# tachitachi/SR-WaveNet

Hardware: AMD Instinct MI355X
Metric: audio samples/sec (fwd+bwd) 30-layer teacher WaveNet (higher is better)
Workload: dtype bf16; 1 GPU; 30-layer teacher WaveNet (3x[1..512] dilations, 64 res / 256 skip ch, 256-way mu-law softmax), fwd+bwd+Adam, batch 8x16000 samples per GPU; global_batch=8, seq_len=16000, parallelism=dp1, launch=hipGraph

## Files before the change

### sr-wavenet_amd/csrc/srwn_wgradt.hip

```cpp
#include "srwn_common.h"
#include "srwn_group.h"
#include "srwn_host.h"
#include "../../include/srwn.h"

using namespace srwn;
using namespace srwn::grp;

namespace {

constexpr int kMaxBlk = 16;
constexpr int kNB = 4;
constexpr int kTileB = 32 * 512;

struct WtBlk { int nl; int layer[4]; int st, W, nsub, KT; };
struct WtSkipArgs {
  const void* cT; long long wt_stride;
  const void* d; long long d_row_stride;
  void* partials; float* bias_partials;
  int part16;
  int B, Tlen, nslabs, mtotal;
  int safe_wait;
  int bias_blk;
  WtBlk blk[kMaxBlk];
};

__device__ uint4 g_zero_row[32];

typedef bf16_t T;

__device__ __forceinline__ f32x4 gload16_untracked(const void* p) {
  f32x4 v;
  asm volatile("global_load_dwordx4 %0, %1, off nt" : "=v"(v) : "v"(p) : "memory");
  return v;
}

struct Cursor {
  int idx, seg, k, wrem;
  long long drow0;
};

__global__ __launch_bounds__(512) void wgrad_skip_wt_kernel(WtSkipArgs a) {
  extern __shared__ __attribute__((aligned(16))) char smem[];
  const int tid = threadIdx.x, lane = tid & 63, wave = __builtin_amdgcn_readfirstlane(tid >> 6);
  const int slab = blockIdx.x;
  const WtBlk& bk = a.blk[blockIdx.y];
  const int st = bk.st, W = bk.W, nsub = bk.nsub, KT = bk.KT;
  const int slot = wave >> 1, nh = wave & 1;
  const bool live = slot < bk.nl;
  const int layer = bk.layer[live ? slot : 0];
  const int per_clip = st * nsub;
  const int nseg = a.B * per_clip;
  const int sps = (nseg + a.nslabs - 1) / a.nslabs;
  const int s0 = slab * sps;
  const int s1 = (s0 + sps < nseg) ? s0 + sps : nseg;
  const int nchunk = (s1 > s0 ? s1 - s0 : 0) * KT;
  const int nit = (nchunk + 2) / 3 * 3;

  auto seg_setup = [&](Cursor& c) {
    const int b = c.seg / per_clip;
    const int rem = c.seg - b * per_clip;
    int r, j0;
    if (nsub == 1) { r = rem; j0 = 0; }
    else { r = rem / nsub; j0 = (rem - r * nsub) * W; }
    const int Jr = (a.Tlen - r + st - 1) / st;
    const int wseg = (Jr - j0) < W ? (Jr - j0) : W;
    c.wrem = wseg;
    c.drow0 = (long long)b * a.Tlen + r + (long long)st * j0;
  };
  auto start = [&](Cursor& c) {
    c.idx = 0; c.seg = nchunk > 0 ? s0 : 0; c.k = 0; c.wrem = 0; c.drow0 = 0;
    if (nchunk > 0) seg_setup(c);
  };
  auto advance = [&](Cursor& c) {
    ++c.idx;
    if (c.idx >= nchunk) { c.wrem = 0; return; }
    ++c.k; c.wrem -= 32;
    if (c.k == KT) { c.k = 0; ++c.seg; seg_setup(c); }
  };

  const int drow_a = 2 * wave + (lane >> 5);
  const int dcol = 32 * ((((lane & 31) >> 1) ^ wave)) + 16 * (lane & 1);
  const char* dbase = reinterpret_cast<const char*>(a.d) + dcol;
  const char* zrow = reinterpret_cast<const char*>(g_zero_row) + dcol;
  const long long drow_bytes = a.d_row_stride * (long long)sizeof(T);
  const unsigned lds0 = (unsigned)(size_t)smem;
  auto dma_tile = [&](const Cursor& c, int buf) {
    const long long row0 = c.drow0 + (long long)st * (32 * c.k);
    const char* ga = (drow_a < c.wrem) ? dbase + (row0 + (long long)st * drow_a) * drow_bytes : zrow;
    const char* gb = (drow_a + 16 < c.wrem) ? dbase + (row0 + (long long)st * (drow_a + 16)) * drow_bytes : zrow;
    const unsigned l = lds0 + buf * kTileB + wave * 1024;
    glds16_untracked(ga, __builtin_amdgcn_readfirstlane(l));
    glds16_untracked(gb, __builtin_amdgcn_readfirstlane(l + 8 * 1024));
  };
  const T* ct_layer = reinterpret_cast<const T*>(a.cT) + (size_t)layer * a.wt_stride + lane * 8;
  auto load_a = [&](const Cursor& c, f32x4 (&f)[4]) {
    const T* t = ct_layer + ((size_t)c.seg * KT + c.k) * (64 * 32);
#pragma unroll
    for (int mb = 0; mb < 4; ++mb) f[mb] = gload16_untracked(t + mb * 512);
  };

  const int kg = lane >> 4, q = (lane & 15) >> 2, p = lane & 3;
  const int hl = ((kg & 1) + 2 * q) & 7;
  const int rowoff = (16 * (kg >> 1) + 2 * (kg & 1) + 4 * q) * 512 + 8 * p;
  int boff[8];
#pragma unroll
  for (int i = 0; i < 8; ++i) boff[i] = rowoff + 32 * (8 * nh + (i ^ hl));

  f32x4 acc[4][8];
#pragma unroll
  for (int mb = 0; mb < 4; ++mb)
#pragma unroll
    for (int i = 0; i < 8; ++i) acc[mb][i] = f32x4{0.f, 0.f, 0.f, 0.f};
  const bool do_bias = a.bias_partials != nullptr && (int)blockIdx.y == a.bias_blk && slot == 3;
  float bsum[8];
#pragma unroll
  for (int i = 0; i < 8; ++i) bsum[i] = 0.0f;
  Frag<T> ones;
#pragma unroll
  for (int j = 0; j < 8; ++j) ones.set(j, 1.0f);

  Cursor ca, cd;
  start(ca); start(cd);
  f32x4 A0[4], A1[4], A2[4];
  dma_tile(cd, 0); advance(cd);
  load_a(ca, A0); advance(ca);
  dma_tile(cd, 1); advance(cd);
  load_a(ca, A1); advance(ca);
  dma_tile(cd, 2); advance(cd);

  typedef short s16x4 __attribute__((ext_vector_type(4)));
  auto bfrag = [&](int buf, int i) {
    const char* bp = smem + buf * kTileB + boff[i];
    s16x4 lo = __builtin_amdgcn_ds_read_tr16_b64_v4i16((__attribute__((address_space(3))) s16x4*)(bp));
    s16x4 hi = __builtin_amdgcn_ds_read_tr16_b64_v4i16((__attribute__((address_space(3))) s16x4*)(bp + 512));
    Frag<T> bf;
    bf.v = __builtin_bit_cast(bf16x8, __builtin_shufflevector(lo, hi, 0, 1, 2, 3, 4, 5, 6, 7));
    return bf;
  };
  Frag<T> bq0 = zero_frag<T>(), bq1 = zero_frag<T>();
  auto compute = [&](int buf, int nbuf, const f32x4 (&A)[4]) {
    Frag<T> af[4];
#pragma unroll
    for (int mb = 0; mb < 4; ++mb) af[mb].v = __builtin_bit_cast(bf16x8, A[mb]);
    Frag<T> b[10];
    b[0] = bq0; b[1] = bq1;
#pragma unroll
    for (int i = 0; i < 8; ++i) {
      b[i + 2] = (i + 2 < 8) ? bfrag(buf, i + 2) : bfrag(nbuf, i + 2 - 8);
#pragma unroll
      for (int mb = 0; mb < 4; ++mb) mma16(acc[mb][i], af[mb], b[i]);
      __builtin_amdgcn_sched_barrier(0);
    }
    bq0 = b[8]; bq1 = b[9];
  };
  auto bias_only = [&](int buf) {
#pragma unroll
    for (int i = 0; i < 8; ++i) bsum[i] = frag_dot(bsum[i], bfrag(buf, i), ones);
  };
#define SRWN_WT_ITER(IT, ACUR, ANEW)                                                                            \
  {                                                                                                             \
        \
    asm volatile("s_waitcnt vmcnt(6)" : "+v"(ACUR[0]), "+v"(ACUR[1]), "+v"(ACUR[2]), "+v"(ACUR[3])::"memory");       \
    if (a.safe_wait) asm volatile("s_waitcnt vmcnt(0)" : "+v"(ACUR[0]), "+v"(ACUR[1]), "+v"(ACUR[2]), "+v"(ACUR[3])::"memory"); \
    wg_barrier();                                                                                               \
    load_a(ca, ANEW); advance(ca);                                                                              \
    dma_tile(cd, ((IT) + 3) & (kNB - 1)); advance(cd);                                                          \
    if (live) compute((IT) & (kNB - 1), ((IT) + 1) & (kNB - 1), ACUR);                                          \
    else if (do_bias) bias_only((IT) & (kNB - 1));                                                              \
  }
  if (nit > 0) {
    if (a.safe_wait) asm volatile("s_waitcnt vmcnt(0)" ::: "memory");
    else asm volatile("s_waitcnt vmcnt(6)" ::: "memory");
    wg_barrier();
    if (live) { bq0 = bfrag(0, 0); bq1 = bfrag(0, 1); }
  }
  for (int it = 0; it < nit; it += 3) {
    SRWN_WT_ITER(it, A0, A2)
    SRWN_WT_ITER(it + 1, A1, A0)
    SRWN_WT_ITER(it + 2, A2, A1)
  }
#undef SRWN_WT_ITER
  asm volatile("s_waitcnt vmcnt(0)" : "+v"(A0[0]), "+v"(A1[0]), "+v"(A2[0])::"memory");

  if (live && a.part16) {
    bf16_t* pb = reinterpret_cast<bf16_t*>(a.partials) + (size_t)slab * a.mtotal * 256;
#pragma unroll
    for (int mb = 0; mb < 4; ++mb)
#pragma unroll
      for (int i = 0; i < 8; ++i) {
        const size_t blk = (size_t)(layer * 4 + mb) * 16 + 8 * nh + i;
        __builtin_nontemporal_store(bf16x4{(bf16_t)acc[mb][i][0], (bf16_t)acc[mb][i][1], (bf16_t)acc[mb][i][2], (bf16_t)acc[mb][i][3]},
                                    reinterpret_cast<bf16x4*>(pb + (blk * 64 + lane) * 4));
      }
  } else if (live) {
    float* pb = reinterpret_cast<float*>(a.partials) + ((size_t)slab * a.mtotal + (size_t)layer * 64) * 256 + 128 * nh + (lane & 15);
#pragma unroll
    for (int mb = 0; mb < 4; ++mb)
#pragma unroll
      for (int i = 0; i < 8; ++i)
#pragma unroll
        for (int r = 0; r < 4; ++r) pb[(size_t)(16 * mb + 4 * (lane >> 4) + r) * 256 + 16 * i] = acc[mb][i][r];
  }
  if (do_bias) {
#pragma unroll
    for (int i = 0; i < 8; ++i) {
      float v = bsum[i];
      v += __shfl_xor(v, 16);
      v += __shfl_xor(v, 32);
      if (lane < 16) a.bias_partials[(size_t)slab * 256 + 128 * nh + 16 * i + lane] = v;
    }
  }
}

__global__ __launch_bounds__(256) void colsum256_kernel(const T* d, long long row_stride, long long rows, int nslabs, float* out) {
  const long long rps = (rows + nslabs - 1) / nslabs;
  const long long r0 = (long long)blockIdx.x * rps;
  const long long r1 = (r0 + rps < rows) ? r0 + rps : rows;
  float s0 = 0.0f, s1 = 0.0f;
  const int c = 2 * (threadIdx.x & 127), half = threadIdx.x >> 7;
  for (long long r = r0 + half; r < r1; r += 2) {
    const unsigned v = *reinterpret_cast<const unsigned*>(d + r * row_stride + c);
    s0 += __builtin_bit_cast(float, v << 16);
    s1 += __builtin_bit_cast(float, v & 0xffff0000u);
  }
  __shared__ float red[2][256];
  red[half][c] = s0; red[half][c + 1] = s1;
  __syncthreads();
  out[(size_t)blockIdx.x * 256 + threadIdx.x] = red[0][threadIdx.x] + red[1][threadIdx.x];
}

int plan_blocks(const int32_t* st, const int32_t* seg_rows, int nlayers, int T, WtBlk* out) {
  int nb = 0;
  bool used[512] = {false};
  if (nlayers > 512) return -1;
  for (int l = 0; l < nlayers; ++l) {
    if (used[l]) continue;
    if (nb == kMaxBlk) return -1;
    WtBlk& b = out[nb++];
    b.nl = 0; b.st = st[l]; b.W = seg_rows[l];
    const int J = (T + b.st - 1) / b.st;
    b.nsub = (J + b.W - 1) / b.W;
    b.KT = (b.W + 31) / 32;
    for (int m = l; m < nlayers && b.nl < 4; ++m)
      if (!used[m] && st[m] == b.st && seg_rows[m] == b.W) { b.layer[b.nl++] = m; used[m] = true; }
    for (int i = b.nl; i < 4; ++i) b.layer[i] = b.layer[0];
  }
  return nb;
}

}

extern "C" int32_t srwn_wgrad_skip_wt_slabs(const int32_t* st, const int32_t* seg_rows, int32_t nlayers, int32_t T) {
  if (!st || !seg_rows || nlayers < 1 || T < 1) return 0;
  for (int l = 0; l < nlayers; ++l) if (st[l] < 1 || seg_rows[l] < 1) return 0;
  WtBlk blk[kMaxBlk];
  const int nb = plan_blocks(st, seg_rows, nlayers, T, blk);
  if (nb < 1) return 0;
  const int s = group_grid() / nb;
  return s < 1 ? 1 : s;
}

extern "C" int srwn_wgrad_skip_wt(const void* cT, int64_t wt_layer_stride, const int32_t* st, const int32_t* seg_rows,
                                  int32_t nlayers, const void* d, int64_t d_row_stride, void* partials,
                                  float* bias_partials, int32_t part16, int32_t nslabs, int32_t B, int32_t T, int32_t R,
                                  int32_t S, int32_t dtype, void* stream) {
  if (B == 0 || T == 0 || nlayers == 0) return 0;
  if (!cT || !st || !seg_rows || !d || !partials) return set_error(SRWN_E_NULL, "wgrad_skip_wt: null pointer");
  if (dtype != SRWN_BF16 || R != 64 || S != 256)
    return set_error(SRWN_E_UNSUPPORTED, "wgrad_skip_wt: built for bf16, 64 residual / 256 skip channels (dtype %d R=%d S=%d)", dtype, R, S);
  if (B < 0 || T < 0 || nlayers < 0 || nslabs < 1 || d_row_stride < S || (d_row_stride % 8) || wt_layer_stride < 0)
    return set_error(SRWN_E_SHAPE, "wgrad_skip_wt: B=%d T=%d layers=%d nslabs=%d d_row_stride=%lld", B, T, nlayers, nslabs,
                     (long long)d_row_stride);
  for (int l = 0; l < nlayers; ++l)
    if (st[l] < 1 || seg_rows[l] < 1) return set_error(SRWN_E_SHAPE, "wgrad_skip_wt: layer %d stride %d segment %d", l, st[l], seg_rows[l]);
  WtSkipArgs a;
  a.cT = cT; a.wt_stride = wt_layer_stride; a.d = d; a.d_row_stride = d_row_stride; a.partials = partials;
  a.part16 = part16 ? 1 : 0;
  a.bias_partials = bias_partials; a.B = B; a.Tlen = T; a.nslabs = nslabs; a.mtotal = nlayers * 64;
  const int nb = plan_blocks(st, seg_rows, nlayers, T, a.blk);
  if (nb < 1) return set_error(SRWN_E_UNSUPPORTED, "wgrad_skip_wt: more than %d layer blocks", kMaxBlk);
  for (int i = 0; i < nb; ++i) {
    const long long nseg = (long long)B * a.blk[i].st * a.blk[i].nsub;
    if (nseg > 0x7fffffffLL || nseg * a.blk[i].KT * 64 * 32 > wt_layer_stride)
      return set_error(SRWN_E_SHAPE, "wgrad_skip_wt: %lld segments x %d tiles exceed wt_layer_stride %lld", nseg, a.blk[i].KT,
                       (long long)wt_layer_stride);
  }
  a.bias_blk = -1;
  a.safe_wait = safe_wait();
  if (bias_partials)
    for (int i = 0; i < nb && a.bias_blk < 0; ++i)
      if (a.blk[i].nl < 4) a.bias_blk = i;
  if (bias_partials && a.bias_blk < 0)
    hipLaunchKernelGGL(colsum256_kernel, dim3((unsigned)nslabs), dim3(256), 0, (hipStream_t)stream,
                       reinterpret_cast<const bf16_t*>(d), (long long)d_row_stride, (long long)B * T, nslabs, bias_partials);
  const size_t sh = (size_t)kNB * kTileB;
  hipError_t e = hipFuncSetAttribute((const void*)wgrad_skip_wt_kernel, hipFuncAttributeMaxDynamicSharedMemorySize, (int)sh);
  if (e != hipSuccess) return set_error((int)e, "wgrad_skip_wt: LDS %zu: %s", sh, hipGetErrorString(e));
  hipLaunchKernelGGL(wgrad_skip_wt_kernel, dim3((unsigned)nslabs, (unsigned)nb), dim3(512), sh, (hipStream_t)stream, a);
  return check_launch("wgrad_skip_wt");
}
```

Before: 80.02 million samples/s.

## Stage A operand through LDS ring with spread DMA issue in wgrad skip kernel

Adds a default LDS mode where the cT (A) operand is DMA'd into a 5-slot LDS ring through global_load_lds instead of being held in three register sets. The next A fragment is read mid-compute, and the tile and A DMA issues are spread between MFMA steps. The aim is to cut register pressure and even out memory issue against the MFMA work. It costs more LDS (about 144KB in total), which may lower occupancy, and adds LDS read traffic. Alternative register modes and debug timestamp instrumentation are also added.

```diff
diff --git a/sr-wavenet_amd/csrc/srwn_wgradt.hip b/sr-wavenet_amd/csrc/srwn_wgradt.hip
--- a/sr-wavenet_amd/csrc/srwn_wgradt.hip
+++ b/sr-wavenet_amd/csrc/srwn_wgradt.hip
@@ -11,6 +11,22 @@
 constexpr int kMaxBlk = 16;
 constexpr int kNB = 4;
 constexpr int kTileB = 32 * 512;
+constexpr int kRing = 5;
+constexpr int kSlotB = 16 * 1024;
+constexpr int kStampB = 2 * 512 * 8;
+enum { kWtRegs3 = 0, kWtRegs4 = 1, kWtLds = 2 };
+#ifndef SRWN_WT_MODE
+#define SRWN_WT_MODE 2
+#endif
+constexpr int kWtMode = SRWN_WT_MODE;
+#ifndef SRWN_WT_SPREAD
+#define SRWN_WT_SPREAD 2
+#endif
+constexpr bool kWtSpread = SRWN_WT_SPREAD != 0;
+constexpr int kWtSpreadAt = SRWN_WT_SPREAD == 2 ? 4 : 0;
+constexpr size_t wt_lds_bytes(int mode, bool stamp) {
+  return (size_t)kNB * kTileB + (mode == kWtLds ? (size_t)kRing * kSlotB : 0) + (stamp ? kStampB : 0);
+}
 
 struct WtBlk { int nl; int layer[4]; int st, W, nsub, KT; };
 struct WtSkipArgs {
@@ -21,6 +37,7 @@
   int B, Tlen, nslabs, mtotal;
   int safe_wait;
   int bias_blk;
+  unsigned long long* stamps;
   WtBlk blk[kMaxBlk];
 };
 
@@ -34,14 +51,36 @@
   return v;
 }
 
+__device__ __forceinline__ void glds16_nt_untracked(const void* g, unsigned lds_addr) {
+  unsigned keep;
+  asm volatile("s_mov_b32 %0, m0\n\ts_mov_b32 m0, %2\n\ts_nop 0\n\tglobal_load_lds_dwordx4 %1, off nt\n\ts_mov_b32 m0, %0"
+               : "=&s"(keep) : "v"(g), "s"(lds_addr) : "memory");
+}
+
+template <bool STAMP> struct WtStamper {
+  unsigned long long* p; int n;
+  __device__ __forceinline__ void operator()(int tag) {
+    if (STAMP && p && n < 512) { p[n] = ((unsigned long long)tag << 48) | (__builtin_amdgcn_s_memtime() & 0xffffffffffffull); ++n; }
+  }
+};
+
 struct Cursor {
   int idx, seg, k, wrem;
   long long drow0;
 };
 
+template <int MODE, bool STAMP>
 __global__ __launch_bounds__(512) void wgrad_skip_wt_kernel(WtSkipArgs a) {
   extern __shared__ __attribute__((aligned(16))) char smem[];
   const int tid = threadIdx.x, lane = tid & 63, wave = __builtin_amdgcn_readfirstlane(tid >> 6);
+  WtStamper<STAMP> stamp{nullptr, 0};
+  const bool stamped = STAMP && blockIdx.x == 0 && blockIdx.y == 0 && (wave & 3) == 0;
+  unsigned long long* const stamp_lds = reinterpret_cast<unsigned long long*>(smem + wt_lds_bytes(MODE, false)) + (wave >> 2) * 512;
+  if (stamped) {
+    for (int i = lane; i < 512; i += 64) stamp_lds[i] = 0;
+    if (lane == 0) stamp.p = stamp_lds;
+  }
+  stamp(1);
   const int slab = blockIdx.x;
   const WtBlk& bk = a.blk[blockIdx.y];
   const int st = bk.st, W = bk.W, nsub = bk.nsub, KT = bk.KT;
@@ -54,7 +93,8 @@
   const int s0 = slab * sps;
   const int s1 = (s0 + sps < nseg) ? s0 + sps : nseg;
   const int nchunk = (s1 > s0 ? s1 - s0 : 0) * KT;
-  const int nit = (nchunk + 2) / 3 * 3;
+  constexpr int kSets = MODE == kWtRegs4 ? 4 : 3;
+  const int nit = MODE == kWtLds ? nchunk : (nchunk + kSets - 1) / kSets * kSets;
 
   auto seg_setup = [&](Cursor& c) {
     const int b = c.seg / per_clip;
@@ -84,17 +124,26 @@
   const char* zrow = reinterpret_cast<const char*>(g_zero_row) + dcol;
   const long long drow_bytes = a.d_row_stride * (long long)sizeof(T);
   const unsigned lds0 = (unsigned)(size_t)smem;
+  const char* dlane_a = dbase + (long long)st * drow_a * drow_bytes;
+  const char* dlane_b = dbase + (long long)st * (drow_a + 16) * drow_bytes;
+  struct TileDma { const char* ga; const char* gb; unsigned l; };
+  auto tile_addr = [&](const Cursor& c, int buf) {
+    const long long tile0 = (c.drow0 + (long long)st * (32 * c.k)) * drow_bytes;
+    TileDma t;
+    t.ga = (drow_a < c.wrem) ? dlane_a + tile0 : zrow;
+    t.gb = (drow_a + 16 < c.wrem) ? dlane_b + tile0 : zrow;
+    t.l = __builtin_amdgcn_readfirstlane(lds0 + buf * kTileB + wave * 1024);
+    return t;
+  };
+  auto dma_half = [&](const TileDma& t, int h) { glds16_untracked(h ? t.gb : t.ga, t.l + h * 8 * 1024); };
   auto dma_tile = [&](const Cursor& c, int buf) {
-    const long long row0 = c.drow0 + (long long)st * (32 * c.k);
-    const char* ga = (drow_a < c.wrem) ? dbase + (row0 + (long long)st * drow_a) * drow_bytes : zrow;
-    const char* gb = (drow_a + 16 < c.wrem) ? dbase + (row0 + (long long)st * (drow_a + 16)) * drow_bytes : zrow;
-    const unsigned l = lds0 + buf * kTileB + wave * 1024;
-    glds16_untracked(ga, __builtin_amdgcn_readfirstlane(l));
-    glds16_untracked(gb, __builtin_amdgcn_readfirstlane(l + 8 * 1024));
+    const TileDma t = tile_addr(c, buf);
+    dma_half(t, 0); dma_half(t, 1);
   };
   const T* ct_layer = reinterpret_cast<const T*>(a.cT) + (size_t)layer * a.wt_stride + lane * 8;
+  auto a_addr = [&](const Cursor& c) { return ct_layer + ((size_t)c.seg * KT + c.k) * (64 * 32); };
   auto load_a = [&](const Cursor& c, f32x4 (&f)[4]) {
-    const T* t = ct_layer + ((size_t)c.seg * KT + c.k) * (64 * 32);
+    const T* t = a_addr(c);
 #pragma unroll
     for (int mb = 0; mb < 4; ++mb) f[mb] = gload16_untracked(t + mb * 512);
   };
@@ -119,14 +168,19 @@
 #pragma unroll
   for (int j = 0; j < 8; ++j) ones.set(j, 1.0f);
 
-  Cursor ca, cd;
-  start(ca); start(cd);
-  f32x4 A0[4], A1[4], A2[4];
-  dma_tile(cd, 0); advance(cd);
-  load_a(ca, A0); advance(ca);
-  dma_tile(cd, 1); advance(cd);
-  load_a(ca, A1); advance(ca);
-  dma_tile(cd, 2); advance(cd);
+  const unsigned ring0 = lds0 + kNB * kTileB;
+  auto dma_c_half = [&](const T* t, int rs, int h) {
+    glds16_nt_untracked(t + nh * 1024 + h * 512, __builtin_amdgcn_readfirstlane(ring0 + rs * kSlotB + wave * 2048 + h * 1024));
+  };
+  auto dma_c = [&](const Cursor& c, int rs) {
+    const T* t = a_addr(c);
+    dma_c_half(t, rs, 0); dma_c_half(t, rs, 1);
+  };
+  auto read_a = [&](int rs, Frag<T> (&f)[4]) {
+    const char* ap = smem + kNB * kTileB + rs * kSlotB + slot * 4096 + lane * 16;
+#pragma unroll
+    for (int mb = 0; mb < 4; ++mb) f[mb].v = *reinterpret_cast<const bf16x8*>(ap + mb * 1024);
+  };
 
   typedef short s16x4 __attribute__((ext_vector_type(4)));
   auto bfrag = [&](int buf, int i) {
@@ -138,18 +192,18 @@
     return bf;
   };
   Frag<T> bq0 = zero_frag<T>(), bq1 = zero_frag<T>();
-  auto compute = [&](int buf, int nbuf, const f32x4 (&A)[4]) {
-    Frag<T> af[4];
-#pragma unroll
-    for (int mb = 0; mb < 4; ++mb) af[mb].v = __builtin_bit_cast(bf16x8, A[mb]);
+  Frag<T> anext[4];
+  auto compute = [&](int buf, int nbuf, const Frag<T> (&af)[4], int nrs, auto&& issue) {
     Frag<T> b[10];
     b[0] = bq0; b[1] = bq1;
 #pragma unroll
     for (int i = 0; i < 8; ++i) {
       b[i + 2] = (i + 2 < 8) ? bfrag(buf, i + 2) : bfrag(nbuf, i + 2 - 8);
+      if (MODE == kWtLds && i == 4) read_a(nrs, anext);
 #pragma unroll
       for (int mb = 0; mb < 4; ++mb) mma16(acc[mb][i], af[mb], b[i]);
       __builtin_amdgcn_sched_barrier(0);
+      if (kWtSpread && i >= kWtSpreadAt) { issue(i - kWtSpreadAt); __builtin_amdgcn_sched_barrier(0); }
     }
     bq0 = b[8]; bq1 = b[9];
   };
@@ -157,30 +211,112 @@
 #pragma unroll
     for (int i = 0; i < 8; ++i) bsum[i] = frag_dot(bsum[i], bfrag(buf, i), ones);
   };
+  auto mfma_done = [&]() {
+    if (STAMP) { asm volatile("" :: "v"(acc[0][7]), "v"(acc[3][7])); stamp(13); }
+  };
+
+  Cursor ca, cd;
+  start(ca); start(cd);
+  if constexpr (MODE == kWtLds) {
+    dma_c(ca, 0); advance(ca);
+    dma_c(ca, 1); advance(ca);
+    dma_tile(cd, 0); advance(cd);
+    dma_c(ca, 2); advance(ca);
+    dma_tile(cd, 1); advance(cd);
+    dma_c(ca, 3); advance(ca);
+    dma_tile(cd, 2); advance(cd);
+    dma_c(ca, 4); advance(ca);
+    if (nit > 0) {
+      if (a.safe_wait) asm volatile("s_waitcnt vmcnt(0)" ::: "memory");
+      else asm volatile("s_waitcnt vmcnt(6)" ::: "memory");
+      wg_barrier();
+      if (live) { bq0 = bfrag(0, 0); bq1 = bfrag(0, 1); read_a(0, anext); }
+    }
+    int rs = 0;
+    for (int it = 0; it < nit; ++it) {
+      const int nrs = rs == kRing - 1 ? 0 : rs + 1;
+      asm volatile("s_waitcnt vmcnt(6)" ::: "memory");
+      if (a.safe_wait) asm volatile("s_waitcnt vmcnt(0)" ::: "memory");
+      stamp(10);
+      wg_barrier();
+      stamp(11);
+      const TileDma td = tile_addr(cd, (it + 3) & (kNB - 1)); advance(cd);
+      const T* ta = a_addr(ca); advance(ca);
+      auto issue = [&](int i) {
+        if (i < 2) dma_half(td, i);
+        else if (i < 4) dma_c_half(ta, rs, i - 2);
+      };
+      if (!kWtSpread || !live) {
+#pragma unroll
+        for (int i = 0; i < 4; ++i) issue(i);
+      }
+      stamp(12);
+      if (live) {
+        Frag<T> af[4];
+#pragma unroll
+        for (int mb = 0; mb < 4; ++mb) af[mb] = anext[mb];
+        compute(it & (kNB - 1), (it + 1) & (kNB - 1), af, nrs, issue);
+      } else if (do_bias) bias_only(it & (kNB - 1));
+      mfma_done();
+      rs = nrs;
+    }
+    asm volatile("s_waitcnt vmcnt(0)" ::: "memory");
+  } else {
+  f32x4 A0[4], A1[4], A2[4], A3[4];
+  dma_tile(cd, 0); advance(cd);
+  load_a(ca, A0); advance(ca);
+  dma_tile(cd, 1); advance(cd);
+  load_a(ca, A1); advance(ca);
+  dma_tile(cd, 2); advance(cd);
+  if (MODE == kWtRegs4) { load_a(ca, A2); advance(ca); }
 #define SRWN_WT_ITER(IT, ACUR, ANEW)                                                                            \
   {                                                                                                             \
         \
-    asm volatile("s_waitcnt vmcnt(6)" : "+v"(ACUR[0]), "+v"(ACUR[1]), "+v"(ACUR[2]), "+v"(ACUR[3])::"memory");       \
+    asm volatile("s_waitcnt vmcnt(%4)" : "+v"(ACUR[0]), "+v"(ACUR[1]), "+v"(ACUR[2]), "+v"(ACUR[3]) : "n"(MODE == kWtRegs4 ? 10 : 6) : "memory"); \
     if (a.safe_wait) asm volatile("s_waitcnt vmcnt(0)" : "+v"(ACUR[0]), "+v"(ACUR[1]), "+v"(ACUR[2]), "+v"(ACUR[3])::"memory"); \
+    stamp(10);                                                                                                  \
     wg_barrier();                                                                                               \
+    stamp(11);                                                                                                  \
+    if (MODE == kWtRegs4) { dma_tile(cd, ((IT) + 3) & (kNB - 1)); advance(cd); }                                \
     load_a(ca, ANEW); advance(ca);                                                                              \
-    dma_tile(cd, ((IT) + 3) & (kNB - 1)); advance(cd);                                                          \
-    if (live) compute((IT) & (kNB - 1), ((IT) + 1) & (kNB - 1), ACUR);                                          \
-    else if (do_bias) bias_only((IT) & (kNB - 1));                                                              \
+    if (MODE != kWtRegs4) { dma_tile(cd, ((IT) + 3) & (kNB - 1)); advance(cd); }                                \
+    stamp(12);                                                                                                  \
+    if (live) {                                                                                                 \
+      Frag<T> af[4];                                                                                            \
+      _Pragma("unroll") for (int mb = 0; mb < 4; ++mb) af[mb].v = __builtin_bit_cast(bf16x8, ACUR[mb]);         \
+      compute((IT) & (kNB - 1), ((IT) + 1) & (kNB - 1), af, 0, [](int) {});                                     \
+    } else if (do_bias) bias_only((IT) & (kNB - 1));                                                            \
+    mfma_done();                                                                                                \
   }
   if (nit > 0) {
     if (a.safe_wait) asm volatile("s_waitcnt vmcnt(0)" ::: "memory");
-    else asm volatile("s_waitcnt vmcnt(6)" ::: "memory");
+    else asm volatile("s_waitcnt vmcnt(%0)" :: "n"(MODE == kWtRegs4 ? 10 : 6) : "memory");
     wg_barrier();
     if (live) { bq0 = bfrag(0, 0); bq1 = bfrag(0, 1); }
   }
-  for (int it = 0; it < nit; it += 3) {
-    SRWN_WT_ITER(it, A0, A2)
-    SRWN_WT_ITER(it + 1, A1, A0)
-    SRWN_WT_ITER(it + 2, A2, A1)
+  if constexpr (MODE == kWtRegs4) {
+    for (int it = 0; it < nit; it += 4) {
+      SRWN_WT_ITER(it, A0, A3)
+      SRWN_WT_ITER(it + 1, A1, A0)
+      SRWN_WT_ITER(it + 2, A2, A1)
+      SRWN_WT_ITER(it + 3, A3, A2)
+    }
+    asm volatile("s_waitcnt vmcnt(0)" : "+v"(A0[0]), "+v"(A1[0]), "+v"(A2[0]), "+v"(A3[0])::"memory");
+  } else {
+    for (int it = 0; it < nit; it += 3) {
+      SRWN_WT_ITER(it, A0, A2)
+      SRWN_WT_ITER(it + 1, A1, A0)
+      SRWN_WT_ITER(it + 2, A2, A1)
+    }
+    asm volatile("s_waitcnt vmcnt(0)" : "+v"(A0[0]), "+v"(A1[0]), "+v"(A2[0])::"memory");
   }
 #undef SRWN_WT_ITER
-  asm volatile("s_waitcnt vmcnt(0)" : "+v"(A0[0]), "+v"(A1[0]), "+v"(A2[0])::"memory");
+  }
+  stamp(2);
+  if (stamped) {
+    unsigned long long* out = a.stamps + (wave >> 2) * 512;
+    for (int i = lane; i < 512; i += 64) out[i] = stamp_lds[i];
+  }
 
   if (live && a.part16) {
     bf16_t* pb = reinterpret_cast<bf16_t*>(a.partials) + (size_t)slab * a.mtotal * 256;
@@ -293,9 +429,12 @@
   if (bias_partials && a.bias_blk < 0)
     hipLaunchKernelGGL(colsum256_kernel, dim3((unsigned)nslabs), dim3(256), 0, (hipStream_t)stream,
                        reinterpret_cast<const bf16_t*>(d), (long long)d_row_stride, (long long)B * T, nslabs, bias_partials);
-  const size_t sh = (size_t)kNB * kTileB;
-  hipError_t e = hipFuncSetAttribute((const void*)wgrad_skip_wt_kernel, hipFuncAttributeMaxDynamicSharedMemorySize, (int)sh);
+  void (*kfn)(WtSkipArgs) = wgrad_skip_wt_kernel<kWtMode, false>;
+  size_t sh = wt_lds_bytes(kWtMode, false);
+  a.stamps = nullptr;
+  SRWN_DIAG_ONLY(if (debug_stamps()) { a.stamps = debug_stamps(); kfn = wgrad_skip_wt_kernel<kWtMode, true>; sh = wt_lds_bytes(kWtMode, true); })
+  hipError_t e = hipFuncSetAttribute((const void*)kfn, hipFuncAttributeMaxDynamicSharedMemorySize, (int)sh);
   if (e != hipSuccess) return set_error((int)e, "wgrad_skip_wt: LDS %zu: %s", sh, hipGetErrorString(e));
-  hipLaunchKernelGGL(wgrad_skip_wt_kernel, dim3((unsigned)nslabs, (unsigned)nb), dim3(512), sh, (hipStream_t)stream, a);
+  hipLaunchKernelGGL(kfn, dim3((unsigned)nslabs, (unsigned)nb), dim3(512), sh, (hipStream_t)stream, a);
   return check_launch("wgrad_skip_wt");
 }
```

New measurement: 80.55 million samples/s, median of 6. About the same (+0.7%).
